# DichenZhang1/libultrahdr_dev

Hardware: AMD Instinct MI355X
Metric: MPixels/sec gain-map generate+apply, 4K P010 batch (higher is better)
Workload: dtype u8/u16 in, f32+f64 math, u8/u32 out

## Files before the change

### libultrahdr_dev_amd/csrc/uhdr_kernels.hip

```cpp
#include "uhdr_kernels.h"

#include <hip/hip_runtime.h>

#include <algorithm>
#include <cmath>

#include "uhdr_device_math.h"
#include "uhdr_wave_scan.h"

namespace uhdr {

__constant__ float c_idw4[4 * 64];

__constant__ float c_idw4p[64];

hipError_t upload_idw4(const float* tables) {
  float p[64];
  for (int oy = 0; oy < 4; ++oy)
    for (int pr = 0; pr < 2; ++pr)
      for (int k = 0; k < 4; ++k)
        for (int h = 0; h < 2; ++h) p[((oy * 2 + pr) * 4 + k) * 2 + h] = tables[oy * 16 + (2 * pr + h) * 4 + k];
  hipError_t e = hipMemcpyToSymbol(HIP_SYMBOL(c_idw4p), p, sizeof(p));
  if (e != hipSuccess) return e;
  return hipMemcpyToSymbol(HIP_SYMBOL(c_idw4), tables, sizeof(float) * 4 * 64);
}

constexpr float k255 = 1 / 255.0f;
constexpr float k876 = 1 / 876.0f;
constexpr float k896 = 1 / 896.0f;

constexpr float kP3YR = 0.299f, kP3YG = 0.587f, kP3YB = 0.114f;
constexpr float kP3Cb = 1.772f, kP3Cr = 1.402f;
constexpr float kP3GCb = kP3YB * kP3Cb / kP3YG;
constexpr float kP3GCr = kP3YR * kP3Cr / kP3YG;

typedef float f2 __attribute__((ext_vector_type(2)));
__device__ __forceinline__ f2 pk_fma(f2 a, f2 b, f2 c) { return __builtin_elementwise_fma(a, b, c); }
__device__ __forceinline__ f2 splat(float v) { return (f2){v, v}; }
__device__ __forceinline__ f2 bc_lo(f2 v) { return __builtin_shufflevector(v, v, 0, 0); }
__device__ __forceinline__ f2 bc_hi(f2 v) { return __builtin_shufflevector(v, v, 1, 1); }

__device__ __forceinline__ f2 pk_add_sat(f2 a, f2 b) {
  f2 r;
  asm("v_pk_add_f32 %0, %1, %2 clamp" : "=v"(r) : "v"(a), "v"(b));
  return r;
}
__device__ __forceinline__ f2 pk_mul_sat(f2 a, f2 b) {
  f2 r;
  asm("v_pk_mul_f32 %0, %1, %2 clamp" : "=v"(r) : "v"(a), "v"(b));
  return r;
}
__device__ __forceinline__ f2 pk_fma_sat(f2 a, f2 b, f2 c) {
  f2 r;
  asm("v_pk_fma_f32 %0, %1, %2, %3 clamp" : "=v"(r) : "v"(a), "v"(b), "v"(c));
  return r;
}

template <int HI>
__device__ __forceinline__ f2 pk_fma_sat_bc(f2 a, f2 b, f2 c) {
  f2 r;
  if (HI) asm("v_pk_fma_f32 %0, %1, %2, %3 op_sel:[0,0,1] op_sel_hi:[1,1,1] clamp" : "=v"(r) : "v"(a), "v"(b), "v"(c));
  else asm("v_pk_fma_f32 %0, %1, %2, %3 op_sel_hi:[1,1,0] clamp" : "=v"(r) : "v"(a), "v"(b), "v"(c));
  return r;
}


__device__ __attribute__((noinline)) uint32_t lut_index_wild(float t) {
  const double pos = (double)t + 0.5;
  uint32_t v = 0u;
  if (__builtin_fabs(pos) < 9223372036854775808.0) v = (uint32_t)(long long)pos;
  return v;
}
__device__ __forceinline__ uint32_t round_half_up(float t) {
  int r;
  asm("v_cvt_rpi_i32_f32 %0, %1" : "=v"(r) : "v"(t));
  return (uint32_t)r;
}
__device__ __forceinline__ uint32_t lut_index(float e, uint32_t n) {
  const float t = e * (float)(n - 1u);
  uint32_t v;
  if (__builtin_expect(__float_as_uint(t) < 0x4F000000u, 1)) v = round_half_up(t);
  else v = lut_index_wild(t);
  return min(v, n - 1u);
}
__device__ __forceinline__ uint32_t lut_index_unit(float e, uint32_t n) {
  return round_half_up(e * (float)(n - 1u));
}
__device__ __forceinline__ float gain_lut_entry(uint32_t idx, double log2_min, double log2_max, float boost_factor) {
  const float value = (float)idx / (float)(kGainLutN - 1u);
  const float log_boost = (float)(log2_min * (double)(1.0f - value) + log2_max * (double)value);
  return (float)exp2((double)(log_boost * boost_factor));
}

__global__ void __launch_bounds__(256) k_build_luts(float* lut) {
  const uint32_t i = blockIdx.x * 256u + threadIdx.x;
  if (i >= kLutTotal) return;
  float y;
  if (i < kLutHlgInv) y = srgb_inv_oetf_exact((float)(i - kLutSrgbInv) / (float)(kLutSrgbInvN - 1u));
  else if (i < kLutPqInv) y = hlg_inv_oetf_exact((float)(i - kLutHlgInv) / (float)(kLutHlgInvN - 1u));
  else if (i < kLutHlg) y = pq_inv_oetf_exact((float)(i - kLutPqInv) / (float)(kLutPqInvN - 1u));
  else if (i < kLutPq) y = hlg_oetf_exact((float)(i - kLutHlg) / (float)(kLutHlgN - 1u));
  else y = pq_oetf_exact((float)(i - kLutPq) / (float)(kLutPqN - 1u));
  lut[i] = y;
}
hipError_t launch_build_luts(float* lut, hipStream_t s) {
  hipLaunchKernelGGL(k_build_luts, dim3((kLutTotal + 255u) / 256u), dim3(256), 0, s, lut);
  return hipGetLastError();
}
__global__ void __launch_bounds__(256) k_build_lut_codes(float* lut) {
  const uint32_t i = blockIdx.x * 256u + threadIdx.x;
  const uint32_t t = i >> 16, k = i & 0xFFFFu;
  uint16_t* codes = reinterpret_cast<uint16_t*>(lut + (t ? kCodePq : kCodeHlg));
  codes[k] = (uint16_t)(0x3ffu & (uint32_t)(lut[(t ? kLutPq : kLutHlg) + k] * 1023.0f));
}
hipError_t launch_build_lut_codes(float* lut, hipStream_t s) {
  hipLaunchKernelGGL(k_build_lut_codes, dim3(2u * 65536u / 256u), dim3(256), 0, s, lut);
  return hipGetLastError();
}
__global__ void __launch_bounds__(256) k_build_gain_lut(float* table, double log2_min, double log2_max, float boost_factor) {
  const uint32_t i = blockIdx.x * 256u + threadIdx.x;
  if (i < kGainLutN) table[i] = gain_lut_entry(i, log2_min, log2_max, boost_factor);
}
hipError_t launch_build_gain_lut(float* table, double log2_min, double log2_max, float boost_factor, hipStream_t s) {
  hipLaunchKernelGGL(k_build_gain_lut, dim3(kGainLutN / 256u), dim3(256), 0, s, table, log2_min, log2_max, boost_factor);
  return hipGetLastError();
}


template <int TF>
__device__ __forceinline__ float hdr_inv_oetf(float e) {
  if (TF == 1) return hlg_inv_oetf_guarded(e);
  if (TF == 2) return pq_inv_oetf_guarded(e);
  return e;
}

__device__ __forceinline__ float cvt_word0(uint32_t w) {
  float r;
  asm("v_cvt_f32_u32_sdwa %0, %1 dst_sel:DWORD dst_unused:UNUSED_PAD src0_sel:WORD_0" : "=v"(r) : "v"(w));
  return r;
}
__device__ __forceinline__ float cvt_word1(uint32_t w) {
  float r;
  asm("v_cvt_f32_u32_sdwa %0, %1 dst_sel:DWORD dst_unused:UNUSED_PAD src0_sel:WORD_1" : "=v"(r) : "v"(w));
  return r;
}


constexpr int kGenWhole = 0, kGenFront = 1, kGenBack = 2, kGenLinear = 3;
struct GenMid { f2 r, g, b, hr, hg, hb; };
template <int TF, bool LUT, bool FILTER, bool DEFER = false, int PART = kGenWhole>
__device__ __forceinline__ uint32_t gen_pair(const GenConsts& c, const uint32_t (&hy)[2][4][2],
                                             const uint32_t (&huv)[2][2][2], const uint32_t (&y8)[2][4],
                                             const uint32_t (&u8)[2][2], const uint32_t (&v8)[2][2],
                                             uint8_t (&out)[2], float (&gain)[2], const float* s_srgb, const float* s_hdr,
                                             GenMid* mid = nullptr) {
  f2 r, g, b, hr, hg, hb;
  if (PART == kGenBack) {
    r = mid->r; g = mid->g; b = mid->b; hr = mid->hr; hg = mid->hg; hb = mid->hb;
  } else {
  f2 sy = splat(0.0f), su = splat(0.0f), sv = splat(0.0f);
  f2 hsy = splat(0.0f), hsu = splat(0.0f), hsv = splat(0.0f);
#pragma unroll
  for (int r = 0; r < 2; ++r) {
    f2 uf[2], vf[2], huf[2], hvf[2];
#pragma unroll
    for (int k = 0; k < 2; ++k) {
      const f2 ub = (f2){(float)((u8[0][r] >> (8 * k)) & 0xffu), (float)((u8[1][r] >> (8 * k)) & 0xffu)};
      const f2 vb = (f2){(float)((v8[0][r] >> (8 * k)) & 0xffu), (float)((v8[1][r] >> (8 * k)) & 0xffu)};
      uf[k] = pk_fma(ub, splat(k255), splat(-128.0f * k255));
      vf[k] = pk_fma(vb, splat(k255), splat(-128.0f * k255));
      const uint32_t m0 = huv[0][r][k] & 0xFFC0FFC0u, m1 = huv[1][r][k] & 0xFFC0FFC0u;
      const f2 hu = (f2){cvt_word0(m0), cvt_word0(m1)};
      const f2 hv = (f2){cvt_word1(m0), cvt_word1(m1)};
      huf[k] = pk_fma(hu, splat(k896 * 0.015625f), splat(-64.0f * k896)) - splat(0.5f);
      hvf[k] = pk_fma(hv, splat(k896 * 0.015625f), splat(-64.0f * k896)) - splat(0.5f);
    }
#pragma unroll
    for (int d = 0; d < 2; ++d) {
      const int dy = 2 * r + d;
#pragma unroll
      for (int dx = 0; dx < 4; ++dx) {
        const f2 yb = (f2){(float)((y8[0][dy] >> (8 * dx)) & 0xffu), (float)((y8[1][dy] >> (8 * dx)) & 0xffu)};
        sy += yb * splat(k255);
        su += uf[dx >> 1];
        sv += vf[dx >> 1];
        const uint32_t w0 = hy[0][dy][dx >> 1] & 0xFFC0FFC0u, w1 = hy[1][dy][dx >> 1] & 0xFFC0FFC0u;
        const f2 hb = (dx & 1) ? (f2){cvt_word1(w0), cvt_word1(w1)} : (f2){cvt_word0(w0), cvt_word0(w1)};
        hsy += pk_fma(hb, splat(k876 * 0.015625f), splat(-64.0f * k876));
        hsu += huf[dx >> 1];
        hsv += hvf[dx >> 1];
      }
    }
  }
  sy *= splat(0.0625f); su *= splat(0.0625f); sv *= splat(0.0625f);
  hsy *= splat(0.0625f); hsu *= splat(0.0625f); hsv *= splat(0.0625f);

  r = pk_add_sat(sy, splat(c.sdr_cr) * sv);
  g = pk_add_sat(sy - splat(c.sdr_gcb) * su, -(splat(c.sdr_gcr) * sv));
  b = pk_add_sat(sy, splat(c.sdr_cb) * su);
  hr = pk_add_sat(hsy, splat(c.hdr_cr) * hsv);
  hg = pk_add_sat(hsy - splat(c.hdr_gcb) * hsu, -(splat(c.hdr_gcr) * hsv));
  hb = pk_add_sat(hsy, splat(c.hdr_cb) * hsu);
  }
  static_assert(PART != kGenLinear || (!LUT && !FILTER), "kGenLinear is the exact path's");
  if (PART != kGenBack && PART != kGenLinear && mid != nullptr) { mid->r = r; mid->g = g; mid->b = b; mid->hr = hr; mid->hg = hg; mid->hb = hb; }
  if (PART == kGenFront) return 0u;

  if (FILTER && !LUT) {
    const f2 fr = (f2){srgb_inv_oetf_fast(r.x), srgb_inv_oetf_fast(r.y)};
    const f2 fg = (f2){srgb_inv_oetf_fast(g.x), srgb_inv_oetf_fast(g.y)};
    const f2 fb = (f2){srgb_inv_oetf_fast(b.x), srgb_inv_oetf_fast(b.y)};
    const f2 fs = (splat(c.lum_r) * fr + splat(c.lum_g) * fg + splat(c.lum_b) * fb) * splat(203.0f);
    f2 qr = hr, qg = hg, qb = hb;
    if (TF == 1) {
      qr = (f2){hlg_inv_oetf_fast(hr.x), hlg_inv_oetf_fast(hr.y)};
      qg = (f2){hlg_inv_oetf_fast(hg.x), hlg_inv_oetf_fast(hg.y)};
      qb = (f2){hlg_inv_oetf_fast(hb.x), hlg_inv_oetf_fast(hb.y)};
    } else if (TF == 2) {
      qr = (f2){pq_inv_oetf_fast(hr.x), pq_inv_oetf_fast(hr.y)};
      qg = (f2){pq_inv_oetf_fast(hg.x), pq_inv_oetf_fast(hg.y)};
      qb = (f2){pq_inv_oetf_fast(hb.x), pq_inv_oetf_fast(hb.y)};
    }
    if (!c.gm_identity) {
      const f2 t0 = splat(c.gm[0]) * qr + splat(c.gm[1]) * qg + splat(c.gm[2]) * qb;
      const f2 t1 = splat(c.gm[3]) * qr + splat(c.gm[4]) * qg + splat(c.gm[5]) * qb;
      const f2 t2 = splat(c.gm[6]) * qr + splat(c.gm[7]) * qg + splat(c.gm[8]) * qb;
      qr = t0; qg = t1; qb = t2;
    }
    const f2 fh = (splat(c.lum_r) * qr + splat(c.lum_g) * qg + splat(c.lum_b) * qb) * splat(c.hdr_white_nits);
    uint32_t fbyte[2], fexact = 0u, doubt = 0u;
    float fgain[2];
#pragma unroll
    for (int k = 0; k < 2; ++k) {
      const float ys = k ? fs.y : fs.x, yh = k ? fh.y : fh.x;
      const float gf = (ys > 0.0f) ? yh * __builtin_amdgcn_rcpf(ys) : 1.0f;
      const float gc = __builtin_amdgcn_fmed3f(gf, c.min_boost, c.max_boost);
      const float v = (__builtin_amdgcn_logf(gc) - c.log2_min) * c.flt_scale;
      const float fl = __builtin_floorf(v), fr2 = v - fl;
      const bool lo = gf < c.flt_lo, hi = gf > c.flt_hi;
      const bool mid = (fr2 >= c.flt_delta) && (fr2 <= 1.0f - c.flt_delta);
      const bool sane = !(ys > 0.0f && ys < 1e-10f) && !(yh != 0.0f && __builtin_fabsf(yh) < 1e-10f);
      if (!((lo || hi || mid) && sane)) doubt |= 1u << k;
      fbyte[k] = lo ? c.enc_byte_min : hi ? c.enc_byte_max : (uint32_t)fl;
      fgain[k] = gf;
      if (!(ys > 0.0f)) fexact |= 1u << k;
    }
    if (DEFER || __builtin_amdgcn_ballot_w64(doubt != 0u) == 0ull) {
      out[0] = (uint8_t)fbyte[0]; out[1] = (uint8_t)fbyte[1];
      gain[0] = fgain[0]; gain[1] = fgain[1];
      return fexact | (doubt << 2);
    }
  }
  constexpr int kLockstep = 6;
  if (LUT) {
    r = (f2){s_srgb[lut_index_unit(r.x, kLutSrgbInvN)], s_srgb[lut_index_unit(r.y, kLutSrgbInvN)]};
    g = (f2){s_srgb[lut_index_unit(g.x, kLutSrgbInvN)], s_srgb[lut_index_unit(g.y, kLutSrgbInvN)]};
    b = (f2){s_srgb[lut_index_unit(b.x, kLutSrgbInvN)], s_srgb[lut_index_unit(b.y, kLutSrgbInvN)]};
  } else {
    float ch[6] = {r.x, r.y, g.x, g.y, b.x, b.y};
#pragma unroll
    for (int i = 0; i < 6; i += kLockstep) {
      float part[kLockstep];
#pragma unroll
      for (int j = 0; j < kLockstep; ++j) part[j] = ch[i + j];
      srgb_inv_oetf_guarded_n<kLockstep>(part);
#pragma unroll
      for (int j = 0; j < kLockstep; ++j) ch[i + j] = part[j];
    }
    r = (f2){ch[0], ch[1]}; g = (f2){ch[2], ch[3]}; b = (f2){ch[4], ch[5]};
  }
  const f2 sdr_nits = (splat(c.lum_r) * r + splat(c.lum_g) * g + splat(c.lum_b) * b) * splat(203.0f);

  if (TF != 0 && LUT) {
    hr = (f2){s_hdr[lut_index_unit(hr.x, kLutHlgInvN)], s_hdr[lut_index_unit(hr.y, kLutHlgInvN)]};
    hg = (f2){s_hdr[lut_index_unit(hg.x, kLutHlgInvN)], s_hdr[lut_index_unit(hg.y, kLutHlgInvN)]};
    hb = (f2){s_hdr[lut_index_unit(hb.x, kLutHlgInvN)], s_hdr[lut_index_unit(hb.y, kLutHlgInvN)]};
  } else if (TF != 0) {
    float ch[6] = {hr.x, hr.y, hg.x, hg.y, hb.x, hb.y};
#pragma unroll
    for (int i = 0; i < 6; i += kLockstep) {
      float part[kLockstep];
#pragma unroll
      for (int j = 0; j < kLockstep; ++j) part[j] = ch[i + j];
      if (TF == 1) hlg_inv_oetf_guarded_n<kLockstep>(part);
      else pq_inv_oetf_guarded_n<kLockstep>(part);
#pragma unroll
      for (int j = 0; j < kLockstep; ++j) ch[i + j] = part[j];
    }
    hr = (f2){ch[0], ch[1]}; hg = (f2){ch[2], ch[3]}; hb = (f2){ch[4], ch[5]};
  }
  if (!c.gm_identity) {
    const f2 t0 = splat(c.gm[0]) * hr + splat(c.gm[1]) * hg + splat(c.gm[2]) * hb;
    const f2 t1 = splat(c.gm[3]) * hr + splat(c.gm[4]) * hg + splat(c.gm[5]) * hb;
    const f2 t2 = splat(c.gm[6]) * hr + splat(c.gm[7]) * hg + splat(c.gm[8]) * hb;
    hr = t0; hg = t1; hb = t2;
  }
  if (PART == kGenLinear) { mid->r = r; mid->g = g; mid->b = b; mid->hr = hr; mid->hg = hg; mid->hb = hb; return 0u; }
  const f2 hdr_nits = (splat(c.lum_r) * hr + splat(c.lum_g) * hg + splat(c.lum_b) * hb) * splat(c.hdr_white_nits);

  gain[0] = raw_gain(sdr_nits.x, hdr_nits.x);
  gain[1] = raw_gain(sdr_nits.y, hdr_nits.y);
#pragma unroll
  for (int k = 0; k < 2; ++k)
    out[k] = encode_gain_guarded(gain[k], c.min_boost, c.max_boost, c.log2_min, c.log2_max, c.enc_scale, c.enc_byte_min,
                                 c.enc_byte_max);
  return 3u;
}

typedef uint32_t u32x4 __attribute__((ext_vector_type(4)));
typedef uint32_t u32x2 __attribute__((ext_vector_type(2)));
__device__ __forceinline__ uint4 ld_stream(const uint4* p) {
  const u32x4 v = __builtin_nontemporal_load(reinterpret_cast<const u32x4*>(p));
  return make_uint4(v.x, v.y, v.z, v.w);
}
__device__ __forceinline__ uint2 ld_stream(const uint2* p) {
  const u32x2 v = __builtin_nontemporal_load(reinterpret_cast<const u32x2*>(p));
  return make_uint2(v.x, v.y);
}
__device__ __forceinline__ uint32_t ld_stream(const uint32_t* p) {
  return __builtin_nontemporal_load(p);
}
__device__ __forceinline__ void st_stream(uint4* p, uint4 v) {
  __builtin_nontemporal_store((u32x4){v.x, v.y, v.z, v.w}, reinterpret_cast<u32x4*>(p));
}
__device__ __forceinline__ void st_stream(uint2* p, uint2 v) {
  __builtin_nontemporal_store((u32x2){v.x, v.y}, reinterpret_cast<u32x2*>(p));
}
__device__ __forceinline__ uint32_t ld8(const uint8_t* p) { return *p; }
__device__ __forceinline__ uint32_t ld16(const uint16_t* p) { return *p; }


template <bool ALIGNED>
__device__ __forceinline__ void load_pair(const GenConsts& c, const GenImage& im, const uint8_t* im_v, uint32_t my, uint32_t pr,
                                          bool two, uint32_t (&hy)[2][4][2], uint32_t (&huv)[2][2][2], uint32_t (&y8)[2][4],
                                          uint32_t (&u8)[2][2], uint32_t (&v8)[2][2]) {
  const uint32_t mx = pr * 2u;
  if (ALIGNED) {
    const uint32_t hoff = 4u * my * im.hy_stride + 8u * pr, yoff = 4u * my * im.y_stride + 8u * pr;
#pragma unroll
    for (int r = 0; r < 4; ++r) {
      const uint4 q = ld_stream(reinterpret_cast<const uint4*>(im.hy + (hoff + r * im.hy_stride)));
      hy[0][r][0] = q.x; hy[0][r][1] = q.y; hy[1][r][0] = q.z; hy[1][r][1] = q.w;
      const uint2 p = ld_stream(reinterpret_cast<const uint2*>(im.y + (yoff + r * im.y_stride)));
      y8[0][r] = p.x; y8[1][r] = p.y;
    }
    const uint32_t huvoff = 2u * my * im.huv_stride + 8u * pr, coff = 2u * my * im.c_stride + 4u * pr;
#pragma unroll
    for (int r = 0; r < 2; ++r) {
      const uint4 q = ld_stream(reinterpret_cast<const uint4*>(im.huv + (huvoff + r * im.huv_stride)));
      huv[0][r][0] = q.x; huv[0][r][1] = q.y; huv[1][r][0] = q.z; huv[1][r][1] = q.w;
      const uint32_t uu = ld_stream(reinterpret_cast<const uint32_t*>(im.u + (coff + r * im.c_stride)));
      const uint32_t vv = ld_stream(reinterpret_cast<const uint32_t*>(im_v + (coff + r * im.c_stride)));
      u8[0][r] = uu & 0xffffu; u8[1][r] = uu >> 16;
      v8[0][r] = vv & 0xffffu; v8[1][r] = vv >> 16;
    }
  } else {
#pragma unroll
    for (int k = 0; k < 2; ++k) {
      const bool on = (k == 0) || two;
      const uint32_t x0 = 4u * (mx + k);
#pragma unroll
      for (int r = 0; r < 4; ++r) {
        const uint16_t* hrow = im.hy + (size_t)(4u * my + r) * im.hy_stride + x0;
        const uint8_t* yrow = im.y + (size_t)(4u * my + r) * im.y_stride + x0;
        hy[k][r][0] = on ? (ld16(hrow) | (ld16(hrow + 1) << 16)) : 0u;
        hy[k][r][1] = on ? (ld16(hrow + 2) | (ld16(hrow + 3) << 16)) : 0u;
        y8[k][r] = on ? (ld8(yrow) | (ld8(yrow + 1) << 8) | (ld8(yrow + 2) << 16) | (ld8(yrow + 3) << 24)) : 0u;
      }
#pragma unroll
      for (int r = 0; r < 2; ++r) {
        const uint16_t* crow = im.huv + (size_t)(2u * my + r) * im.huv_stride + x0;
        const uint8_t* urow = im.u + (size_t)(2u * my + r) * im.c_stride + (x0 >> 1);
        const uint8_t* vrow = im_v + (size_t)(2u * my + r) * im.c_stride + (x0 >> 1);
        huv[k][r][0] = on ? (ld16(crow) | (ld16(crow + 1) << 16)) : 0u;
        huv[k][r][1] = on ? (ld16(crow + 2) | (ld16(crow + 3) << 16)) : 0u;
        u8[k][r] = on ? (ld8(urow) | (ld8(urow + 1) << 8)) : 0u;
        v8[k][r] = on ? (ld8(vrow) | (ld8(vrow + 1) << 8)) : 0u;
      }
    }
  }
}

template <int CTRL, int ROWS>
__device__ __forceinline__ float dpp_move(float v) {
  return __int_as_float(__builtin_amdgcn_update_dpp(__float_as_int(v), __float_as_int(v), CTRL, ROWS, 0xF, false));
}
template <bool MAX>
__device__ __forceinline__ float wave_extreme(float v) {
#define UHDR_EXT(CTRL, ROWS) v = MAX ? fmaxf(v, dpp_move<CTRL, ROWS>(v)) : fminf(v, dpp_move<CTRL, ROWS>(v))
  UHDR_EXT(0xB1, 0xF);
  UHDR_EXT(0x4E, 0xF);
  UHDR_EXT(0x141, 0xF);
  UHDR_EXT(0x140, 0xF);
  UHDR_EXT(0x142, 0xA);
  UHDR_EXT(0x143, 0xC);
#undef UHDR_EXT
  return __int_as_float(__builtin_amdgcn_readlane(__float_as_int(v), 63));
}
__device__ __forceinline__ void wave_minmax(float& vmin, float& vmax) {
  vmin = wave_extreme<false>(vmin);
  vmax = wave_extreme<true>(vmax);
}
__device__ __forceinline__ void publish_minmax(float gmin, float gmax, uint32_t* keys) {
  if ((threadIdx.x & 63u) == 0u && gmin <= gmax) {
    const uint32_t kmin = ~float_to_key(gmin), kmax = float_to_key(gmax);
    if (__hip_atomic_load(&keys[0], __ATOMIC_RELAXED, __HIP_MEMORY_SCOPE_AGENT) < kmin) atomicMax(&keys[0], kmin);
    if (__hip_atomic_load(&keys[1], __ATOMIC_RELAXED, __HIP_MEMORY_SCOPE_AGENT) < kmax) atomicMax(&keys[1], kmax);
  }
}

template <int TF, bool ALIGNED, bool LUT>
__device__ __forceinline__ void exact_pair(const GenConsts& c, const GenImage& im, const uint8_t* im_v, uint32_t my,
                                           uint32_t pr, bool two, const float* s_srgb, const float* s_hdr, uint8_t (&o)[2], float (&gn)[2]) {
  uint32_t hy[2][4][2], huv[2][2][2], y8[2][4], u8[2][2], v8[2][2];
  load_pair<ALIGNED>(c, im, im_v, my, pr, two, hy, huv, y8, u8, v8);
  gen_pair<TF, LUT, false>(c, hy, huv, y8, u8, v8, o, gn, s_srgb, s_hdr);
}


template <int TF, bool ALIGNED, bool LUT, bool FILTER, int TILES, bool DEFER, int BLOCK = kGenBlock>
__global__ void __launch_bounds__(BLOCK, 1) k_generate(const GenConsts c, const GenBatch b) {
  __shared__ float s_srgb[LUT ? kLutSrgbInvN : 1];
  __shared__ float s_hdr[(LUT && TF != 0) ? kLutHlgInvN : 1];
  __shared__ float s_kept[(FILTER && DEFER) ? TILES * 2 * BLOCK : 1];
  if (LUT) {
    for (uint32_t i = threadIdx.x; i < kLutSrgbInvN / 4u; i += BLOCK)
      reinterpret_cast<float4*>(s_srgb)[i] = reinterpret_cast<const float4*>(c.lut + kLutSrgbInv)[i];
    if (TF != 0) {
      const float4* src = reinterpret_cast<const float4*>(c.lut + (TF == 1 ? kLutHlgInv : kLutPqInv));
      for (uint32_t i = threadIdx.x; i < kLutHlgInvN / 4u; i += BLOCK) reinterpret_cast<float4*>(s_hdr)[i] = src[i];
    }
    __syncthreads();
  }
  const uint32_t img_i = blockIdx.x, blk = blockIdx.y;
  const GenImage& im = b.img[img_i];
  const uint8_t* im_v = im.u + (size_t)im.c_stride * (c.height / 2u);
  const uint32_t pairs_per_row = (c.map_w + 1u) >> 1;
  const uint32_t total = pairs_per_row * c.map_h;
  const bool stats = c.stat_keys != nullptr;
  float emin = __builtin_inff(), emax = -__builtin_inff();
  float amin = __builtin_inff(), amax = -__builtin_inff();
  uint32_t kept_exact = 0u, kept_valid = 0u, kept_doubt = 0u;
  uint32_t n_saved = 0u;
  uint32_t* wslot = (FILTER && DEFER && c.stat_slots != 0u)
                        ? c.stat_ws + (size_t)kStatWords * blockIdx.x + kStatHdr + (blockIdx.y * (uint32_t)(BLOCK / 64) + (threadIdx.x >> 6)) * kStatSlotWords
                        : nullptr;

#pragma unroll 1
  for (uint32_t t = 0; t < (uint32_t)TILES; ++t) {
    const uint32_t idx = (blk * (uint32_t)TILES + t) * (uint32_t)BLOCK + threadIdx.x;
    if (idx >= total) break;
    const uint32_t my = idx / pairs_per_row;
    const uint32_t pr = idx - my * pairs_per_row;
    const uint32_t mx = pr * 2u;
    const bool two = ALIGNED || (mx + 1u < c.map_w);

    uint32_t hy[2][4][2], huv[2][2][2], y8[2][4], u8[2][2], v8[2][2];
    load_pair<ALIGNED>(c, im, im_v, my, pr, two, hy, huv, y8, u8, v8);

    uint8_t o[2];
    float gn[2];
    GenMid mid;
    const uint32_t ex = gen_pair<TF, LUT, FILTER, DEFER>(c, hy, huv, y8, u8, v8, o, gn, s_srgb, s_hdr, (FILTER && DEFER) ? &mid : nullptr);
    const uint8_t o0 = o[0], o1 = o[1];
    if (FILTER && DEFER) {
      uint32_t dm = (ex >> 2) & (two ? 3u : 1u);
      if (c.stat_slots != 0u) {
        const unsigned long long dmask = __builtin_amdgcn_ballot_w64(dm != 0u);
        if (dmask != 0ull) {
          const uint32_t pos = n_saved + (uint32_t)__builtin_popcountll(dmask & ((1ull << (threadIdx.x & 63u)) - 1ull));
          n_saved += (uint32_t)__builtin_popcountll(dmask);
          if (dm != 0u && pos < kStatSlotSaved) {
            float4* e = reinterpret_cast<float4*>(wslot + 16u + pos * 16u);
            e[0] = make_float4(__uint_as_float((idx << 3) | dm), mid.r.x, mid.r.y, mid.g.x);
            e[1] = make_float4(mid.g.y, mid.b.x, mid.b.y, mid.hr.x);
            e[2] = make_float4(mid.hr.y, mid.hg.x, mid.hg.y, mid.hb.x);
            e[3] = make_float4(mid.hb.y, 0.0f, 0.0f, 0.0f);
            dm = 0u;
          }
        }
      }
      kept_doubt |= dm << (2u * t);
      if (stats) {
        s_kept[(2u * t) * BLOCK + threadIdx.x] = gn[0];
        s_kept[(2u * t + 1u) * BLOCK + threadIdx.x] = gn[1];
        const uint32_t valid = (two ? 3u : 1u) & ~((ex >> 2) & 3u);
        kept_exact |= (ex & 3u) << (2u * t);
        kept_valid |= valid << (2u * t);
        if (valid & 1u) { amin = fminf(amin, gn[0]); amax = fmaxf(amax, gn[0]); }
        if (valid & 2u) { amin = fminf(amin, gn[1]); amax = fmaxf(amax, gn[1]); }
        if (ex & valid & 1u) { emin = fminf(emin, gn[0]); emax = fmaxf(emax, gn[0]); }
        if (ex & valid & 2u) { emin = fminf(emin, gn[1]); emax = fmaxf(emax, gn[1]); }
      }
    } else {
      emin = fminf(emin, gn[0]); emax = fmaxf(emax, gn[0]);
      if (two) { emin = fminf(emin, gn[1]); emax = fmaxf(emax, gn[1]); }
    }
    uint8_t* mp = im.map + (size_t)my * c.map_w + mx;
    if (ALIGNED) {
      *reinterpret_cast<uint16_t*>(mp) = (uint16_t)(o0 | ((uint32_t)o1 << 8));
    } else {
      mp[0] = o0;
      if (two) mp[1] = o1;
    }
  }
  if (FILTER && !DEFER) return;
  if (!FILTER && !stats) return;
  uint32_t* keys = stats ? c.stat_keys + (size_t)c.stat_stride * img_i : nullptr;

  if (FILTER) {
    uint32_t* ws = c.stat_ws + (size_t)kStatWords * img_i;
    uint32_t cand = 0u;
    if (stats) {
      wave_minmax(amin, amax);
      float wmin = emin, wmax = emax;
      wave_minmax(wmin, wmax);
      const float e = c.flt_gain_rel;
      uint32_t* est = c.stat_spread != 0u ? ws + kStatEst + 2u * (blk % kStatLists) : ws;
      uint32_t e0 = __hip_atomic_load(&est[0], __ATOMIC_RELAXED, __HIP_MEMORY_SCOPE_AGENT);
      uint32_t e1 = __hip_atomic_load(&est[1], __ATOMIC_RELAXED, __HIP_MEMORY_SCOPE_AGENT);
      const uint32_t k0 = __hip_atomic_load(&keys[0], __ATOMIC_RELAXED, __HIP_MEMORY_SCOPE_AGENT);
      const uint32_t k1 = __hip_atomic_load(&keys[1], __ATOMIC_RELAXED, __HIP_MEMORY_SCOPE_AGENT);
      if (amin <= amax) {
        const uint32_t m0 = ~float_to_key(amin), m1 = float_to_key(amax);
        if ((threadIdx.x & 63u) == 0u) {
          if (e0 < m0) atomicMax(&est[0], m0);
          if (e1 < m1) atomicMax(&est[1], m1);
        }
        e0 = e0 < m0 ? m0 : e0; e1 = e1 < m1 ? m1 : e1;
      }
      float min_hi = fminf(k1 != 0u ? key_to_float(~k0) : __builtin_inff(), wmin);
      float max_lo = fmaxf(k1 != 0u ? key_to_float(k1) : -__builtin_inff(), wmax);
      if (e1 != 0u) {
        const float pmin = key_to_float(~e0), pmax = key_to_float(e1);
        min_hi = fminf(min_hi, pmin + e * __builtin_fabsf(pmin));
        max_lo = fmaxf(max_lo, pmax - e * __builtin_fabsf(pmax));
      }
#pragma unroll
      for (uint32_t t = 0; t < (uint32_t)TILES; ++t)
#pragma unroll
        for (uint32_t k = 0; k < 2u; ++k) {
          const uint32_t bit = 1u << (2u * t + k);
          if ((kept_valid & bit) && !(kept_exact & bit)) {
            const float a = s_kept[(2u * t + k) * BLOCK + threadIdx.x], slack = e * __builtin_fabsf(a);
            if ((a - slack <= min_hi) || (a + slack >= max_lo)) cand |= 1u << t;
          }
        }
    }
    unsigned long long mask[TILES];
    uint32_t total = 0u;
#pragma unroll
    for (uint32_t t = 0; t < (uint32_t)TILES; ++t) {
      mask[t] = __builtin_amdgcn_ballot_w64((((kept_doubt >> (2u * t)) & 3u) | ((cand >> t) & 1u)) != 0u);
      total += (uint32_t)__builtin_popcountll(mask[t]);
    }
    if (total != 0u || c.stat_slots != 0u) {
      const uint32_t lane = threadIdx.x & 63u, list = blk % kStatLists;
      uint32_t base = 0u, cap = kStatCap;
      uint32_t* lw = ws + kStatHdr + list * kStatCap;
      if (c.stat_slots != 0u) {
        lw = wslot;
        const bool over = total > kStatSlotPlain;
        const uint32_t ns = n_saved < kStatSlotSaved ? n_saved : kStatSlotSaved;
        if (lane == 0u) {
          ws[kStatSlotCnt + blk * (uint32_t)(BLOCK / 64) + (threadIdx.x >> 6)] = over ? 0u : (total | (ns << 8));
          if (over) __hip_atomic_store(&ws[6], 1u, __ATOMIC_RELAXED, __HIP_MEMORY_SCOPE_AGENT);
        }
        ++lw;
        cap = over ? 0u : kStatSlotPlain;
      } else {
        if (lane == 0u) base = atomicAdd(&ws[8u + list], total);
        base = (uint32_t)__builtin_amdgcn_readfirstlane((int)base);
      }
#pragma unroll
      for (uint32_t t = 0; t < (uint32_t)TILES; ++t) {
        const uint32_t flags = ((kept_doubt >> (2u * t)) & 3u) | (((cand >> t) & 1u) << 2);
        const uint32_t pos = base + (uint32_t)__builtin_popcountll(mask[t] & ((1ull << lane) - 1ull));
        if (flags != 0u && pos < cap) lw[pos] = (((blk * (uint32_t)TILES + t) * (uint32_t)BLOCK + threadIdx.x) << 3) | flags;
        base += (uint32_t)__builtin_popcountll(mask[t]);
      }
    }
    if (!stats) return;
  }
  wave_minmax(emin, emax);
  publish_minmax(emin, emax, keys);
}

__global__ void k_stats_finalize(uint32_t* keys, int n) {
  const int i = blockIdx.x * blockDim.x + threadIdx.x;
  if (i >= n) return;
  const uint32_t k0 = keys[2 * i], k1 = keys[2 * i + 1];
  float mn = __builtin_inff(), mx = -__builtin_inff();
  if (k1 != 0u) { mn = key_to_float(~k0); mx = key_to_float(k1); }
  keys[2 * i] = __float_as_uint(mn);
  keys[2 * i + 1] = __float_as_uint(mx);
}

static_assert(kStatLists == 64u, "k_generate_resolve reads the list counts with one wave");
template <int TF, bool ALIGNED>
__global__ void __launch_bounds__(256) k_generate_resolve(const GenConsts c, const GenBatch b) {
  const uint32_t img_i = blockIdx.x;
  const GenImage& im = b.img[img_i];
  const uint8_t* im_v = im.u + (size_t)im.c_stride * (c.height / 2u);
  uint32_t* ws = c.stat_ws + (size_t)kStatWords * img_i;
  const uint32_t pairs_per_row = (c.map_w + 1u) >> 1, total = pairs_per_row * c.map_h;
  const bool stats = c.stat_out != nullptr;
  float emin = __builtin_inff(), emax = -__builtin_inff();
  __shared__ uint32_t s_first[kStatSlotWaves + 1u];
  __shared__ uint8_t s_ns[kStatSlotWaves];
  __shared__ uint32_t s_sweep;
  const bool slots = c.stat_slots != 0u;
  if (slots) {
    static_assert(kStatSlotWaves == 4u * 256u, "four waves' counts per thread");
    __shared__ uint32_t s_part[4];
    uint32_t n4[4];
    const uint4 cw4 = *reinterpret_cast<const uint4*>(ws + kStatSlotCnt + 4u * threadIdx.x);
    const uint32_t cws[4] = {cw4.x, cw4.y, cw4.z, cw4.w};
#pragma unroll
    for (uint32_t j = 0; j < 4u; ++j) {
      const uint32_t w = 4u * threadIdx.x + j;
      const uint32_t cw = w < c.stat_slots ? cws[j] : 0u;
      s_ns[w] = (uint8_t)(cw >> 8);
      n4[j] = (cw & 0xFFu) + (cw >> 8);
    }
    const uint32_t over = __hip_atomic_load(&ws[6], __ATOMIC_RELAXED, __HIP_MEMORY_SCOPE_AGENT);
    const uint32_t mine = n4[0] + n4[1] + n4[2] + n4[3];
    const uint32_t before = block_exclusive_sum<256>(mine, s_part);
    s_first[4u * threadIdx.x] = before;
    s_first[4u * threadIdx.x + 1u] = before + n4[0];
    s_first[4u * threadIdx.x + 2u] = before + n4[0] + n4[1];
    s_first[4u * threadIdx.x + 3u] = before + n4[0] + n4[1] + n4[2];
    if (threadIdx.x == 255u) { s_first[kStatSlotWaves] = before + mine; s_sweep = over; }
  } else if (threadIdx.x < 64u) {
    const uint32_t cnt = ws[8u + threadIdx.x];
    const bool over = __builtin_amdgcn_ballot_w64(cnt > kStatCap) != 0ull;
    uint32_t inc = min(cnt, kStatCap);
#pragma unroll
    for (int off = 1; off < 64; off <<= 1) {
      const uint32_t v = (uint32_t)__shfl_up((int)inc, off, 64);
      if ((int)threadIdx.x >= off) inc += v;
    }
    s_first[threadIdx.x + 1u] = inc;
    if (threadIdx.x == 0) { s_first[0] = 0u; s_sweep = over ? 1u : 0u; }
  }
  __syncthreads();
  const bool sweep = s_sweep != 0u;
  const uint32_t nl = slots ? kStatSlotWaves : kStatLists;
  const uint32_t n = sweep ? total : s_first[nl];
#pragma unroll 1
  for (uint32_t g = blockIdx.y * 256u + threadIdx.x; g < n; g += kResolveSlices * 256u) {
    uint32_t entry = (g << 3) | 7u;
    GenMid mid;
    bool have = false;
    if (!sweep) {
      uint32_t l = 0u;
      for (uint32_t s2 = nl / 2u; s2 != 0u; s2 >>= 1) if (s_first[l + s2] <= g) l += s2;
      const uint32_t k = g - s_first[l];
      if (!slots) {
        entry = ws[kStatHdr + l * kStatCap + k];
      } else if (k >= (uint32_t)s_ns[l]) {
        entry = ws[kStatHdr + l * kStatSlotWords + 1u + (k - (uint32_t)s_ns[l])];
      } else {
        const uint4* e = reinterpret_cast<const uint4*>(ws + kStatHdr + l * kStatSlotWords + 16u + k * 16u);
        const uint4 e0 = e[0], e1 = e[1], e2 = e[2], e3 = e[3];
        entry = e0.x;
        mid.r = (f2){__uint_as_float(e0.y), __uint_as_float(e0.z)};
        mid.g = (f2){__uint_as_float(e0.w), __uint_as_float(e1.x)};
        mid.b = (f2){__uint_as_float(e1.y), __uint_as_float(e1.z)};
        mid.hr = (f2){__uint_as_float(e1.w), __uint_as_float(e2.x)};
        mid.hg = (f2){__uint_as_float(e2.y), __uint_as_float(e2.z)};
        mid.hb = (f2){__uint_as_float(e2.w), __uint_as_float(e3.x)};
        have = true;
      }
    }
    const uint32_t idx = entry >> 3;
    const uint32_t my = idx / pairs_per_row, pr = idx - my * pairs_per_row;
    const bool two = ALIGNED || (pr * 2u + 1u < c.map_w);
    uint8_t o[2];
    float gn[2];
    uint32_t hy[2][4][2], huv[2][2][2], y8[2][4], u8[2][2], v8[2][2];
    if (!have) {
      load_pair<ALIGNED>(c, im, im_v, my, pr, two, hy, huv, y8, u8, v8);
      gen_pair<TF, false, false, false, kGenFront>(c, hy, huv, y8, u8, v8, o, gn, nullptr, nullptr, &mid);
    }
    gen_pair<TF, false, false, false, kGenBack>(c, hy, huv, y8, u8, v8, o, gn, nullptr, nullptr, &mid);
    uint8_t* mp = im.map + (size_t)my * c.map_w + 2u * pr;
    if (entry & 1u) mp[0] = o[0];
    if ((entry & 2u) && two) mp[1] = o[1];
    if ((entry & 5u) != 0u) { emin = fminf(emin, gn[0]); emax = fmaxf(emax, gn[0]); }
    if ((entry & 6u) != 0u && two) { emin = fminf(emin, gn[1]); emax = fmaxf(emax, gn[1]); }
  }
  if (stats) {
    wave_minmax(emin, emax);
    publish_minmax(emin, emax, ws + 4);
  }
  __shared__ uint32_t s_last;
  asm volatile("s_waitcnt vmcnt(0)" ::: "memory");
  __syncthreads();
  if (threadIdx.x == 0) s_last = atomicAdd(&ws[3], 1u);
  __syncthreads();
  if (s_last == kResolveSlices - 1u && threadIdx.x == 0) {
    if (stats) {
      const uint32_t k0 = __hip_atomic_load(&ws[4], __ATOMIC_RELAXED, __HIP_MEMORY_SCOPE_AGENT);
      const uint32_t k1 = __hip_atomic_load(&ws[5], __ATOMIC_RELAXED, __HIP_MEMORY_SCOPE_AGENT);
      float mn = __builtin_inff(), mx = -__builtin_inff();
      if (k1 != 0u) { mn = key_to_float(~k0); mx = key_to_float(k1); }
      c.stat_out[2u * img_i] = mn;
      c.stat_out[2u * img_i + 1u] = mx;
    }
  }
  __syncthreads();
  static_assert(kStatSlotCnt <= 256u, "one header word per thread");
  if (s_last == kResolveSlices - 1u && threadIdx.x < kStatSlotCnt)
    __hip_atomic_store(&ws[threadIdx.x], 0u, __ATOMIC_RELAXED, __HIP_MEMORY_SCOPE_AGENT);
}
template <int TF>
static hipError_t launch_stats_resolve_tf(const GenConsts& c, const GenBatch& b, int n, bool aligned, hipStream_t s) {
  if (aligned) hipLaunchKernelGGL((k_generate_resolve<TF, true>), dim3((unsigned)n, kResolveSlices), dim3(256), 0, s, c, b);
  else hipLaunchKernelGGL((k_generate_resolve<TF, false>), dim3((unsigned)n, kResolveSlices), dim3(256), 0, s, c, b);
  return hipGetLastError();
}
hipError_t launch_stats_resolve(const GenConsts& c, const GenBatch& b, int n, int hdr_tf, bool aligned, hipStream_t s) {
  if (n <= 0 || c.stat_ws == nullptr) return hipSuccess;
  switch (hdr_tf) {
    case 0: return launch_stats_resolve_tf<0>(c, b, n, aligned, s);
    case 1: return launch_stats_resolve_tf<1>(c, b, n, aligned, s);
    case 2: return launch_stats_resolve_tf<2>(c, b, n, aligned, s);
    default: return hipErrorInvalidValue;
  }
}

bool generate_is_small(const GenConsts& c, int n) {
  const uint32_t total = ((c.map_w + 1u) >> 1) * c.map_h;
  const uint32_t span = (uint32_t)kGenBlock * (uint32_t)kGenTiles;
  return (uint64_t)((total + span - 1u) / span) * (uint64_t)n < 1024u;
}

uint32_t generate_slot_waves(const GenConsts& c, int n) {
  const uint32_t total = ((c.map_w + 1u) >> 1) * c.map_h;
  const uint32_t per = (uint32_t)kGenBlock * (generate_is_small(c, n) ? 1u : (uint32_t)kGenTiles);
  const uint64_t waves = (uint64_t)((total + per - 1u) / per) * (uint64_t)(kGenBlock / 64);
  return waves <= kStatSlotWaves ? (uint32_t)waves : 0u;
}

bool generate_resolve_pays(const GenConsts& c, int n) {
  const uint32_t total = ((c.map_w + 1u) >> 1) * c.map_h;
  const uint32_t span = (uint32_t)kGenBlock * (uint32_t)kGenTiles;
  return (uint64_t)((total + span - 1u) / span) * (uint64_t)n >= 128u;
}

template <int TF, bool ALIGNED, bool LUT, bool FILTER>
static hipError_t launch_generate_t(const GenConsts& c, const GenBatch& b, int n, hipStream_t s) {
  const uint32_t total = ((c.map_w + 1u) >> 1) * c.map_h;
  if (total == 0 || n == 0) return hipSuccess;
  const bool small = generate_is_small(c, n);
  const unsigned b4 = (total + (uint32_t)kGenBlock * (uint32_t)kGenTiles - 1u) / ((uint32_t)kGenBlock * (uint32_t)kGenTiles);
  const unsigned b1 = (total + kGenBlock - 1u) / kGenBlock;
  const dim3 g4 = dim3((unsigned)n, b4, 1);
  const dim3 g1 = dim3((unsigned)n, b1, 1);
  if (FILTER) {
    if (c.stat_ws != nullptr) {
      if (small) hipLaunchKernelGGL((k_generate<TF, ALIGNED, LUT, FILTER, 1, true>), g1, dim3(kGenBlock, 1, 1), 0, s, c, b);
      else hipLaunchKernelGGL((k_generate<TF, ALIGNED, LUT, FILTER, kGenTiles, true>), g4, dim3(kGenBlock, 1, 1), 0, s, c, b);
    } else {
      if (c.stat_keys != nullptr) return hipErrorInvalidValue;
      const unsigned h1 = (total + 127u) / 128u;
      if ((uint64_t)h1 * (uint64_t)n >= 2000u) {
        const dim3 gh = dim3((unsigned)n, h1, 1);
        hipLaunchKernelGGL((k_generate<TF, ALIGNED, LUT, FILTER, 1, false, 128>), gh, dim3(128, 1, 1), 0, s, c, b);
      } else {
        hipLaunchKernelGGL((k_generate<TF, ALIGNED, LUT, FILTER, 1, false>), g1, dim3(kGenBlock, 1, 1), 0, s, c, b);
      }
    }
  } else if (small) {
    hipLaunchKernelGGL((k_generate<TF, ALIGNED, LUT, FILTER, 1, false>), g1, dim3(kGenBlock, 1, 1), 0, s, c, b);
  } else {
    hipLaunchKernelGGL((k_generate<TF, ALIGNED, LUT, FILTER, kGenTiles, false>), g4, dim3(kGenBlock, 1, 1), 0, s, c, b);
  }
  return hipGetLastError();
}

template <int TF>
static hipError_t launch_generate_tf(const GenConsts& c, const GenBatch& b, int n, bool aligned, bool lut, bool filter,
                                     hipStream_t s) {
  if (lut) return aligned ? launch_generate_t<TF, true, true, false>(c, b, n, s) : launch_generate_t<TF, false, true, false>(c, b, n, s);
  if (filter && aligned) return launch_generate_t<TF, true, false, true>(c, b, n, s);
  return aligned ? launch_generate_t<TF, true, false, false>(c, b, n, s) : launch_generate_t<TF, false, false, false>(c, b, n, s);
}
hipError_t launch_generate(const GenConsts& c, const GenBatch& b, int n, int hdr_tf, bool aligned, bool lut,
                           bool filter, hipStream_t s) {
  if (lut && c.lut == nullptr) return hipErrorInvalidValue;
  switch (hdr_tf) {
    case 0: return launch_generate_tf<0>(c, b, n, aligned, lut, filter, s);
    case 1: return launch_generate_tf<1>(c, b, n, aligned, lut, filter, s);
    case 2: return launch_generate_tf<2>(c, b, n, aligned, lut, filter, s);
    default: return hipErrorInvalidValue;
  }
}

hipError_t launch_stats_init(uint32_t* keys, int n, hipStream_t s) {
  return hipMemsetAsync(keys, 0, sizeof(uint32_t) * 2 * (size_t)n, s);
}
hipError_t launch_stats_finalize(uint32_t* keys, int n, hipStream_t s) {
  if (n == 0) return hipSuccess;
  hipLaunchKernelGGL(k_stats_finalize, dim3((n + 63) / 64), dim3(64), 0, s, keys, n);
  return hipGetLastError();
// ... 2416 lines not shown
```

Before: 542,600.

## Keep uniform constants in SGPRs, pack gain math, strength-reduce tile address computation

Forces uniform constants and flags into scalar registers via asm constraints and readfirstlane, so the compiler treats them as wave-uniform. Computes the reciprocal, log and floor for the filter path as packed pairs. Replaces the per-tile integer division and address recomputation with incremental row/pair and byte-offset updates. Swaps branchy min/max for bare v_min/v_max with NaN sentinels, and canonicalizes values before the wave reduction. This targets VALU and SALU instruction count and VGPR pressure in the generation loop. It relies on NaN-ignoring hardware min/max semantics, and changes the early break to a continue.

```diff
diff --git a/libultrahdr_dev_amd/csrc/uhdr_kernels.hip b/libultrahdr_dev_amd/csrc/uhdr_kernels.hip
--- a/libultrahdr_dev_amd/csrc/uhdr_kernels.hip
+++ b/libultrahdr_dev_amd/csrc/uhdr_kernels.hip
@@ -37,6 +37,25 @@
 typedef float f2 __attribute__((ext_vector_type(2)));
 __device__ __forceinline__ f2 pk_fma(f2 a, f2 b, f2 c) { return __builtin_elementwise_fma(a, b, c); }
 __device__ __forceinline__ f2 splat(float v) { return (f2){v, v}; }
+__device__ __forceinline__ f2 splat_s(float v) {
+  asm volatile("" : "+s"(v));
+  return (f2){v, v};
+}
+__device__ __forceinline__ bool flag_s(uint32_t v) {
+  v = (uint32_t)__builtin_amdgcn_readfirstlane((int)v);
+  asm volatile("" : "+s"(v));
+  return v != 0u;
+}
+__device__ __forceinline__ float fmin_bare(float a, float b) {
+  float r;
+  asm("v_min_f32 %0, %1, %2" : "=v"(r) : "v"(a), "v"(b));
+  return r;
+}
+__device__ __forceinline__ float fmax_bare(float a, float b) {
+  float r;
+  asm("v_max_f32 %0, %1, %2" : "=v"(r) : "v"(a), "v"(b));
+  return r;
+}
 __device__ __forceinline__ f2 bc_lo(f2 v) { return __builtin_shufflevector(v, v, 0, 0); }
 __device__ __forceinline__ f2 bc_hi(f2 v) { return __builtin_shufflevector(v, v, 1, 1); }
 
@@ -195,12 +214,12 @@
   sy *= splat(0.0625f); su *= splat(0.0625f); sv *= splat(0.0625f);
   hsy *= splat(0.0625f); hsu *= splat(0.0625f); hsv *= splat(0.0625f);
 
-  r = pk_add_sat(sy, splat(c.sdr_cr) * sv);
-  g = pk_add_sat(sy - splat(c.sdr_gcb) * su, -(splat(c.sdr_gcr) * sv));
-  b = pk_add_sat(sy, splat(c.sdr_cb) * su);
-  hr = pk_add_sat(hsy, splat(c.hdr_cr) * hsv);
-  hg = pk_add_sat(hsy - splat(c.hdr_gcb) * hsu, -(splat(c.hdr_gcr) * hsv));
-  hb = pk_add_sat(hsy, splat(c.hdr_cb) * hsu);
+  r = pk_add_sat(sy, splat_s(c.sdr_cr) * sv);
+  g = pk_add_sat(sy - splat_s(c.sdr_gcb) * su, -(splat_s(c.sdr_gcr) * sv));
+  b = pk_add_sat(sy, splat_s(c.sdr_cb) * su);
+  hr = pk_add_sat(hsy, splat_s(c.hdr_cr) * hsv);
+  hg = pk_add_sat(hsy - splat_s(c.hdr_gcb) * hsu, -(splat_s(c.hdr_gcr) * hsv));
+  hb = pk_add_sat(hsy, splat_s(c.hdr_cb) * hsu);
   }
   static_assert(PART != kGenLinear || (!LUT && !FILTER), "kGenLinear is the exact path's");
   if (PART != kGenBack && PART != kGenLinear && mid != nullptr) { mid->r = r; mid->g = g; mid->b = b; mid->hr = hr; mid->hg = hg; mid->hb = hb; }
@@ -210,7 +229,7 @@
     const f2 fr = (f2){srgb_inv_oetf_fast(r.x), srgb_inv_oetf_fast(r.y)};
     const f2 fg = (f2){srgb_inv_oetf_fast(g.x), srgb_inv_oetf_fast(g.y)};
     const f2 fb = (f2){srgb_inv_oetf_fast(b.x), srgb_inv_oetf_fast(b.y)};
-    const f2 fs = (splat(c.lum_r) * fr + splat(c.lum_g) * fg + splat(c.lum_b) * fb) * splat(203.0f);
+    const f2 fs = (splat_s(c.lum_r) * fr + splat_s(c.lum_g) * fg + splat_s(c.lum_b) * fb) * splat(203.0f);
     f2 qr = hr, qg = hg, qb = hb;
     if (TF == 1) {
       qr = (f2){hlg_inv_oetf_fast(hr.x), hlg_inv_oetf_fast(hr.y)};
@@ -221,29 +240,35 @@
       qg = (f2){pq_inv_oetf_fast(hg.x), pq_inv_oetf_fast(hg.y)};
       qb = (f2){pq_inv_oetf_fast(hb.x), pq_inv_oetf_fast(hb.y)};
     }
-    if (!c.gm_identity) {
-      const f2 t0 = splat(c.gm[0]) * qr + splat(c.gm[1]) * qg + splat(c.gm[2]) * qb;
-      const f2 t1 = splat(c.gm[3]) * qr + splat(c.gm[4]) * qg + splat(c.gm[5]) * qb;
-      const f2 t2 = splat(c.gm[6]) * qr + splat(c.gm[7]) * qg + splat(c.gm[8]) * qb;
+    if (!flag_s((uint32_t)c.gm_identity)) {
+      const f2 t0 = splat_s(c.gm[0]) * qr + splat_s(c.gm[1]) * qg + splat_s(c.gm[2]) * qb;
+      const f2 t1 = splat_s(c.gm[3]) * qr + splat_s(c.gm[4]) * qg + splat_s(c.gm[5]) * qb;
+      const f2 t2 = splat_s(c.gm[6]) * qr + splat_s(c.gm[7]) * qg + splat_s(c.gm[8]) * qb;
       qr = t0; qg = t1; qb = t2;
     }
-    const f2 fh = (splat(c.lum_r) * qr + splat(c.lum_g) * qg + splat(c.lum_b) * qb) * splat(c.hdr_white_nits);
+    const f2 fh = (splat_s(c.lum_r) * qr + splat_s(c.lum_g) * qg + splat_s(c.lum_b) * qb) * splat_s(c.hdr_white_nits);
     uint32_t fbyte[2], fexact = 0u, doubt = 0u;
     float fgain[2];
+    const f2 prod = fh * (f2){__builtin_amdgcn_rcpf(fs.x), __builtin_amdgcn_rcpf(fs.y)};
+    const bool lit[2] = {fs.x > 0.0f, fs.y > 0.0f};
+    const f2 gf2 = (f2){lit[0] ? prod.x : 1.0f, lit[1] ? prod.y : 1.0f};
+    const f2 lg = (f2){__builtin_amdgcn_logf(__builtin_amdgcn_fmed3f(gf2.x, c.min_boost, c.max_boost)),
+                       __builtin_amdgcn_logf(__builtin_amdgcn_fmed3f(gf2.y, c.min_boost, c.max_boost))};
+    const f2 v2 = (lg - splat_s(c.log2_min)) * splat_s(c.flt_scale);
+    const f2 fl2 = (f2){__builtin_floorf(v2.x), __builtin_floorf(v2.y)};
+    const f2 frac = v2 - fl2;
+    const float delta_hi = 1.0f - c.flt_delta;
 #pragma unroll
     for (int k = 0; k < 2; ++k) {
       const float ys = k ? fs.y : fs.x, yh = k ? fh.y : fh.x;
-      const float gf = (ys > 0.0f) ? yh * __builtin_amdgcn_rcpf(ys) : 1.0f;
-      const float gc = __builtin_amdgcn_fmed3f(gf, c.min_boost, c.max_boost);
-      const float v = (__builtin_amdgcn_logf(gc) - c.log2_min) * c.flt_scale;
-      const float fl = __builtin_floorf(v), fr2 = v - fl;
+      const float gf = k ? gf2.y : gf2.x, fl = k ? fl2.y : fl2.x, fr2 = k ? frac.y : frac.x;
       const bool lo = gf < c.flt_lo, hi = gf > c.flt_hi;
-      const bool mid = (fr2 >= c.flt_delta) && (fr2 <= 1.0f - c.flt_delta);
-      const bool sane = !(ys > 0.0f && ys < 1e-10f) && !(yh != 0.0f && __builtin_fabsf(yh) < 1e-10f);
+      const bool mid = (fr2 >= c.flt_delta) && (fr2 <= delta_hi);
+      const bool sane = !(lit[k] && ys < 1e-10f) && !(yh != 0.0f && __builtin_fabsf(yh) < 1e-10f);
       if (!((lo || hi || mid) && sane)) doubt |= 1u << k;
       fbyte[k] = lo ? c.enc_byte_min : hi ? c.enc_byte_max : (uint32_t)fl;
       fgain[k] = gf;
-      if (!(ys > 0.0f)) fexact |= 1u << k;
+      if (!lit[k]) fexact |= 1u << k;
     }
     if (DEFER || __builtin_amdgcn_ballot_w64(doubt != 0u) == 0ull) {
       out[0] = (uint8_t)fbyte[0]; out[1] = (uint8_t)fbyte[1];
@@ -269,7 +294,7 @@
     }
     r = (f2){ch[0], ch[1]}; g = (f2){ch[2], ch[3]}; b = (f2){ch[4], ch[5]};
   }
-  const f2 sdr_nits = (splat(c.lum_r) * r + splat(c.lum_g) * g + splat(c.lum_b) * b) * splat(203.0f);
+  const f2 sdr_nits = (splat_s(c.lum_r) * r + splat_s(c.lum_g) * g + splat_s(c.lum_b) * b) * splat(203.0f);
 
   if (TF != 0 && LUT) {
     hr = (f2){s_hdr[lut_index_unit(hr.x, kLutHlgInvN)], s_hdr[lut_index_unit(hr.y, kLutHlgInvN)]};
@@ -290,13 +315,13 @@
     hr = (f2){ch[0], ch[1]}; hg = (f2){ch[2], ch[3]}; hb = (f2){ch[4], ch[5]};
   }
   if (!c.gm_identity) {
-    const f2 t0 = splat(c.gm[0]) * hr + splat(c.gm[1]) * hg + splat(c.gm[2]) * hb;
-    const f2 t1 = splat(c.gm[3]) * hr + splat(c.gm[4]) * hg + splat(c.gm[5]) * hb;
-    const f2 t2 = splat(c.gm[6]) * hr + splat(c.gm[7]) * hg + splat(c.gm[8]) * hb;
+    const f2 t0 = splat_s(c.gm[0]) * hr + splat_s(c.gm[1]) * hg + splat_s(c.gm[2]) * hb;
+    const f2 t1 = splat_s(c.gm[3]) * hr + splat_s(c.gm[4]) * hg + splat_s(c.gm[5]) * hb;
+    const f2 t2 = splat_s(c.gm[6]) * hr + splat_s(c.gm[7]) * hg + splat_s(c.gm[8]) * hb;
     hr = t0; hg = t1; hb = t2;
   }
   if (PART == kGenLinear) { mid->r = r; mid->g = g; mid->b = b; mid->hr = hr; mid->hg = hg; mid->hb = hb; return 0u; }
-  const f2 hdr_nits = (splat(c.lum_r) * hr + splat(c.lum_g) * hg + splat(c.lum_b) * hb) * splat(c.hdr_white_nits);
+  const f2 hdr_nits = (splat_s(c.lum_r) * hr + splat_s(c.lum_g) * hg + splat_s(c.lum_b) * hb) * splat_s(c.hdr_white_nits);
 
   gain[0] = raw_gain(sdr_nits.x, hdr_nits.x);
   gain[1] = raw_gain(sdr_nits.y, hdr_nits.y);
@@ -330,21 +355,36 @@
 __device__ __forceinline__ uint32_t ld16(const uint16_t* p) { return *p; }
 
 
+struct GenOffs { uint32_t h, y, huv, c, m; };
+__device__ __forceinline__ GenOffs gen_offsets(const GenConsts& c, const GenImage& im, uint32_t my, uint32_t pr) {
+  return GenOffs{8u * my * im.hy_stride + 16u * pr, 4u * my * im.y_stride + 8u * pr, 2u * my * im.huv_stride + 8u * pr,
+                 2u * my * im.c_stride + 4u * pr, my * c.map_w + 2u * pr};
+}
+__device__ __forceinline__ void gen_offsets_advance(const GenConsts& c, const GenImage& im, GenOffs& o, uint32_t rows, uint32_t rem,
+                                                    uint32_t pairs_per_row, uint32_t stay) {
+  const uint32_t ph = 8u * im.hy_stride, py = 4u * im.y_stride, phuv = 2u * im.huv_stride, pc = 2u * im.c_stride, pm = c.map_w;
+  o.h += (rows * ph + 16u * rem + (ph - 16u * pairs_per_row)) + ((16u * pairs_per_row - ph) & stay);
+  o.y += (rows * py + 8u * rem + (py - 8u * pairs_per_row)) + ((8u * pairs_per_row - py) & stay);
+  o.huv += (rows * phuv + 8u * rem + (phuv - 8u * pairs_per_row)) + ((8u * pairs_per_row - phuv) & stay);
+  o.c += (rows * pc + 4u * rem + (pc - 4u * pairs_per_row)) + ((4u * pairs_per_row - pc) & stay);
+  o.m += (rows * pm + 2u * rem + (pm - 2u * pairs_per_row)) + ((2u * pairs_per_row - pm) & stay);
+}
 template <bool ALIGNED>
 __device__ __forceinline__ void load_pair(const GenConsts& c, const GenImage& im, const uint8_t* im_v, uint32_t my, uint32_t pr,
                                           bool two, uint32_t (&hy)[2][4][2], uint32_t (&huv)[2][2][2], uint32_t (&y8)[2][4],
-                                          uint32_t (&u8)[2][2], uint32_t (&v8)[2][2]) {
+                                          uint32_t (&u8)[2][2], uint32_t (&v8)[2][2], const GenOffs* at = nullptr) {
   const uint32_t mx = pr * 2u;
   if (ALIGNED) {
-    const uint32_t hoff = 4u * my * im.hy_stride + 8u * pr, yoff = 4u * my * im.y_stride + 8u * pr;
+    const GenOffs o = at != nullptr ? *at : gen_offsets(c, im, my, pr);
+    const uint32_t hoff = o.h, yoff = o.y;
 #pragma unroll
     for (int r = 0; r < 4; ++r) {
-      const uint4 q = ld_stream(reinterpret_cast<const uint4*>(im.hy + (hoff + r * im.hy_stride)));
+      const uint4 q = ld_stream(reinterpret_cast<const uint4*>(reinterpret_cast<const uint8_t*>(im.hy) + (hoff + r * (2u * im.hy_stride))));
       hy[0][r][0] = q.x; hy[0][r][1] = q.y; hy[1][r][0] = q.z; hy[1][r][1] = q.w;
       const uint2 p = ld_stream(reinterpret_cast<const uint2*>(im.y + (yoff + r * im.y_stride)));
       y8[0][r] = p.x; y8[1][r] = p.y;
     }
-    const uint32_t huvoff = 2u * my * im.huv_stride + 8u * pr, coff = 2u * my * im.c_stride + 4u * pr;
+    const uint32_t huvoff = o.huv, coff = o.c;
 #pragma unroll
     for (int r = 0; r < 2; ++r) {
       const uint4 q = ld_stream(reinterpret_cast<const uint4*>(im.huv + (huvoff + r * im.huv_stride)));
@@ -387,6 +427,7 @@
 }
 template <bool MAX>
 __device__ __forceinline__ float wave_extreme(float v) {
+  v = __builtin_canonicalizef(v);
 #define UHDR_EXT(CTRL, ROWS) v = MAX ? fmaxf(v, dpp_move<CTRL, ROWS>(v)) : fminf(v, dpp_move<CTRL, ROWS>(v))
   UHDR_EXT(0xB1, 0xF);
   UHDR_EXT(0x4E, 0xF);
@@ -438,6 +479,7 @@
   const uint32_t pairs_per_row = (c.map_w + 1u) >> 1;
   const uint32_t total = pairs_per_row * c.map_h;
   const bool stats = c.stat_keys != nullptr;
+  const uint32_t stats_word = (uint32_t)((uintptr_t)c.stat_keys | ((uintptr_t)c.stat_keys >> 32));
   float emin = __builtin_inff(), emax = -__builtin_inff();
   float amin = __builtin_inff(), amax = -__builtin_inff();
   uint32_t kept_exact = 0u, kept_valid = 0u, kept_doubt = 0u;
@@ -446,17 +488,21 @@
                         ? c.stat_ws + (size_t)kStatWords * blockIdx.x + kStatHdr + (blockIdx.y * (uint32_t)(BLOCK / 64) + (threadIdx.x >> 6)) * kStatSlotWords
                         : nullptr;
 
+  const uint32_t idx0 = blk * (uint32_t)TILES * (uint32_t)BLOCK + threadIdx.x;
+  uint32_t my = idx0 / pairs_per_row;
+  uint32_t pr = idx0 - my * pairs_per_row;
+  const uint32_t span_rows = TILES > 1 ? (uint32_t)BLOCK / pairs_per_row : 0u;
+  const uint32_t span_rem = TILES > 1 ? (uint32_t)BLOCK - span_rows * pairs_per_row : 0u;
+  GenOffs at = gen_offsets(c, im, my, pr);
 #pragma unroll 1
   for (uint32_t t = 0; t < (uint32_t)TILES; ++t) {
-    const uint32_t idx = (blk * (uint32_t)TILES + t) * (uint32_t)BLOCK + threadIdx.x;
-    if (idx >= total) break;
-    const uint32_t my = idx / pairs_per_row;
-    const uint32_t pr = idx - my * pairs_per_row;
+    const uint32_t idx = idx0 + t * (uint32_t)BLOCK;
+    if (idx >= total) continue;
     const uint32_t mx = pr * 2u;
     const bool two = ALIGNED || (mx + 1u < c.map_w);
 
     uint32_t hy[2][4][2], huv[2][2][2], y8[2][4], u8[2][2], v8[2][2];
-    load_pair<ALIGNED>(c, im, im_v, my, pr, two, hy, huv, y8, u8, v8);
+    load_pair<ALIGNED>(c, im, im_v, my, pr, two, hy, huv, y8, u8, v8, &at);
 
     uint8_t o[2];
     float gn[2];
@@ -465,7 +511,7 @@
     const uint8_t o0 = o[0], o1 = o[1];
     if (FILTER && DEFER) {
       uint32_t dm = (ex >> 2) & (two ? 3u : 1u);
-      if (c.stat_slots != 0u) {
+      if (flag_s(c.stat_slots)) {
         const unsigned long long dmask = __builtin_amdgcn_ballot_w64(dm != 0u);
         if (dmask != 0ull) {
           const uint32_t pos = n_saved + (uint32_t)__builtin_popcountll(dmask & ((1ull << (threadIdx.x & 63u)) - 1ull));
@@ -481,27 +527,35 @@
         }
       }
       kept_doubt |= dm << (2u * t);
-      if (stats) {
+      if (flag_s(stats_word)) {
         s_kept[(2u * t) * BLOCK + threadIdx.x] = gn[0];
         s_kept[(2u * t + 1u) * BLOCK + threadIdx.x] = gn[1];
         const uint32_t valid = (two ? 3u : 1u) & ~((ex >> 2) & 3u);
         kept_exact |= (ex & 3u) << (2u * t);
         kept_valid |= valid << (2u * t);
-        if (valid & 1u) { amin = fminf(amin, gn[0]); amax = fmaxf(amax, gn[0]); }
-        if (valid & 2u) { amin = fminf(amin, gn[1]); amax = fmaxf(amax, gn[1]); }
-        if (ex & valid & 1u) { emin = fminf(emin, gn[0]); emax = fmaxf(emax, gn[0]); }
-        if (ex & valid & 2u) { emin = fminf(emin, gn[1]); emax = fmaxf(emax, gn[1]); }
+        const float skip = __builtin_nanf("");
+        const float a0 = (valid & 1u) ? gn[0] : skip, a1 = (valid & 2u) ? gn[1] : skip;
+        const float e0 = (ex & valid & 1u) ? gn[0] : skip, e1 = (ex & valid & 2u) ? gn[1] : skip;
+        amin = fmin_bare(fmin_bare(amin, a0), a1); amax = fmax_bare(fmax_bare(amax, a0), a1);
+        emin = fmin_bare(fmin_bare(emin, e0), e1); emax = fmax_bare(fmax_bare(emax, e0), e1);
       }
     } else {
-      emin = fminf(emin, gn[0]); emax = fmaxf(emax, gn[0]);
-      if (two) { emin = fminf(emin, gn[1]); emax = fmaxf(emax, gn[1]); }
-    }
-    uint8_t* mp = im.map + (size_t)my * c.map_w + mx;
+      emin = fmin_bare(emin, gn[0]); emax = fmax_bare(emax, gn[0]);
+      if (two) { emin = fmin_bare(emin, gn[1]); emax = fmax_bare(emax, gn[1]); }
+    }
+    uint8_t* mp = ALIGNED ? im.map + at.m : im.map + (size_t)my * c.map_w + mx;
     if (ALIGNED) {
       *reinterpret_cast<uint16_t*>(mp) = (uint16_t)(o0 | ((uint32_t)o1 << 8));
     } else {
       mp[0] = o0;
       if (two) mp[1] = o1;
+    }
+    if (TILES > 1) {
+      const uint32_t over = pr + span_rem - pairs_per_row;
+      const uint32_t stay = (uint32_t)((int32_t)over >> 31);
+      pr = over + (pairs_per_row & stay);
+      my += span_rows + 1u + stay;
+      if (ALIGNED) gen_offsets_advance(c, im, at, span_rows, span_rem, pairs_per_row, stay);
     }
   }
   if (FILTER && !DEFER) return;
```

After: 543,400 (median of 6 runs). About the same (+0.1%).
